# DCASE-REPO/DESED_task

Measured on AMD Instinct MI355X. Metric: 10s-clips/sec CRNN mean-teacher train @batch48, higher is better.
Workload: dtype f32 (fp32 storage and accumulation; the dense contractions of the wide layers run as split-bf16 MFMA, 3 bf16 products per fp32 product, fp32-level accuracy; everything else exact f32)

## Files before the change

### desed_task_amd/csrc/sed_conv.hip

```cpp
#include "sed_common.h"

__global__ __launch_bounds__(256) void pack_weights_kernel(const float* __restrict__ W, float* __restrict__ Wf,
                                                           float* __restrict__ Wd, int COUT, int CIN) {
    const int i = blockIdx.x * 256 + threadIdx.x;
    if (i >= COUT * CIN * 9) return;
    const int b = i % 3, a = (i / 3) % 3, ci = (i / 9) % CIN, co = i / (9 * CIN);
    const float w = W[i];
    Wf[((a * 3 + b) * CIN + ci) * COUT + co] = w;
    if (Wd) Wd[(((2 - a) * 3 + (2 - b)) * COUT + co) * CIN + ci] = w;
}
SED_API int sed_conv_pack_weights(const float* W, float* Wf, float* Wd, int COUT, int CIN, void* stream) {
    const int n = COUT * CIN * 9;
    SED_LAUNCH(pack_weights_kernel, dim3((n + 255) / 256), dim3(256), 0, (hipStream_t)stream, W, Wf, Wd, COUT, CIN);
    return sed_check_launch();
}
struct PackJobs {
    const float* W[8];
    float* Wf[8];
    float* Wd[8];
    int cout[8], cin[8], start[9];
    int n;
};
__global__ __launch_bounds__(256) void pack_weights_multi_kernel(PackJobs jobs) {
    const int i = blockIdx.x * 256 + threadIdx.x;
    if (i >= jobs.start[jobs.n]) return;
    int j = 0;
#pragma unroll
    for (int q = 1; q < 8; ++q) j += (q < jobs.n && i >= jobs.start[q]) ? 1 : 0;
    const int e = i - jobs.start[j], COUT = jobs.cout[j], CIN = jobs.cin[j];
    const int b = e % 3, a = (e / 3) % 3, ci = (e / 9) % CIN, co = e / (9 * CIN);
    const float w = jobs.W[j][e];
    jobs.Wf[j][((a * 3 + b) * CIN + ci) * COUT + co] = w;
    if (jobs.Wd[j]) jobs.Wd[j][(((2 - a) * 3 + (2 - b)) * COUT + co) * CIN + ci] = w;
}
SED_API int sed_conv_pack_multi(int n, const void* const* W, void* const* Wf, void* const* Wd, const int* cout, const int* cin,
                                   void* stream) {
    if (n < 1 || n > 8) return SED_ERR_ARG;
    PackJobs jobs;
    int tot = 0;
    for (int j = 0; j < n; ++j) {
        jobs.W[j] = (const float*)W[j]; jobs.Wf[j] = (float*)Wf[j]; jobs.Wd[j] = Wd ? (float*)Wd[j] : nullptr;
        jobs.cout[j] = cout[j]; jobs.cin[j] = cin[j]; jobs.start[j] = tot;
        tot += cout[j] * cin[j] * 9;
    }
    for (int j = n; j < 8; ++j) { jobs.W[j] = nullptr; jobs.Wf[j] = nullptr; jobs.Wd[j] = nullptr; jobs.cout[j] = 0; jobs.cin[j] = 0; jobs.start[j] = tot; }
    jobs.start[n] = tot;
    jobs.start[8] = tot;
    jobs.n = n;
    SED_LAUNCH(pack_weights_multi_kernel, dim3((tot + 255) / 256), dim3(256), 0, (hipStream_t)stream, jobs);
    return sed_check_launch();
}

__global__ __launch_bounds__(1024) void wgrad_reduce_kernel(const float* __restrict__ parts, float* __restrict__ dW, int nparts,
                                                            int COUT, int CIN) {
    __shared__ float4 red[64][16];
    const int tid = threadIdx.x, col = tid & 15, grp = tid >> 4, G = blockDim.x >> 4;
    const int j = blockIdx.x * 64 + 4 * col;
    const int n = 9 * CIN * COUT;
    float4 acc = make_float4(0.f, 0.f, 0.f, 0.f);
    if (j < n) {
#pragma unroll 4
        for (int p = grp; p < nparts; p += G) {
            const float4 v = *(const float4*)(parts + (size_t)p * n + j);
            acc.x += v.x; acc.y += v.y; acc.z += v.z; acc.w += v.w;
        }
    }
    red[grp][col] = acc;
    __syncthreads();
    if (grp == 0 && j < n) {
        for (int g = 1; g < G; ++g) { const float4 v = red[g][col]; acc.x += v.x; acc.y += v.y; acc.z += v.z; acc.w += v.w; }
        const int co = j % COUT, ci = (j / COUT) % CIN, tap = j / (COUT * CIN);
        float* d = dW + ((size_t)co * CIN + ci) * 9 + tap;
        d[0] = acc.x; d[(size_t)CIN * 9] = acc.y; d[(size_t)2 * CIN * 9] = acc.z; d[(size_t)3 * CIN * 9] = acc.w;
    }
}
static inline int wgrad_parts(int CIN, int COUT, int B, int T, int F) {
    if (CIN <= 32) {
        const int TF = F >= 32 ? 32 : F, TR = 128 / TF;
        const int ntiles = B * ((T + TR - 1) / TR) * (F / TF);
        int cap = CIN <= 16 ? 1024 : 512;
        if (sed_tuning[SED_TUNE_WGRAD_CAP] > 0) cap = sed_tuning[SED_TUNE_WGRAD_CAP];
        return ntiles < cap ? ntiles : cap;
    }
    const int ntiles = (B * T * F + 63) / 64;
    return ntiles < 56 ? ntiles : 56;
}
static inline bool wgrad_row_ok(int CIN, int COUT, int F) {
    return F >= 8 && 64 % F == 0 && COUT == 128 && (CIN == 64 || CIN == 128);
}
static inline int wgrad_row_parts(int CIN, int B, int T, int F) {
    const int ntiles = (B * T * F + 63) / 64, cap = CIN == 64 ? 168 : 84;
    return ntiles < cap ? ntiles : cap;
}
SED_API long long sed_conv_wgrad_scratch_floats(int B, int T, int F, int CIN, int COUT) {
    int parts = wgrad_parts(CIN, COUT, B, T, F);
    if (wgrad_row_ok(CIN, COUT, F) && wgrad_row_parts(CIN, B, T, F) > parts) parts = wgrad_row_parts(CIN, B, T, F);
    return (long long)parts * 9 * CIN * COUT;
}

#define CONV_THREADS(COUT) ((COUT) >= 64 ? 512 : 256)

template <int CIN, int COUT, int TF, int MP = 128>
struct ConvCfg {
    static constexpr int TR = MP / TF;
    static constexpr int PW = TF + 2, PH = TR + 2, PP = PW * PH;
    static constexpr int CK = CIN < 32 ? CIN : 32;
    static constexpr int CKP = CK + 1;
    static constexpr int NCH = CIN / CK;
    static constexpr int NT = (COUT + 31) / 32;
    static constexpr int WM = MP / 32;
    static constexpr int THREADS = CONV_THREADS(COUT);
    static constexpr int WN = THREADS / 64 / WM;
    static constexpr int NTW = NT / WN;
    static_assert(NTW >= 1 && NTW * WN == NT, "wave split must tile COUT");
    static constexpr int WCH = CK * COUT;
    static constexpr int PATCH_F = (PP * CKP + 3) & ~3;
    static constexpr int SMEM = (PATCH_F + 2 * WCH) * 4;
};

template <int CIN, int COUT, int TF, bool STATS, int MP = 128>
__global__ __launch_bounds__(CONV_THREADS(COUT)) void conv3x3_kernel(const float* __restrict__ x, const float* __restrict__ Wp,
                                                      const float* __restrict__ bias, float* __restrict__ y,
                                                      float* __restrict__ partial, int B, int T, int F) {
    using Cfg = ConvCfg<CIN, COUT, TF, MP>;
    constexpr int TR = Cfg::TR, PW = Cfg::PW, PP = Cfg::PP, CK = Cfg::CK, CKP = Cfg::CKP, NCH = Cfg::NCH, NT = Cfg::NT,
                  WCH = Cfg::WCH, NTW = Cfg::NTW, THREADS = Cfg::THREADS, WM = Cfg::WM;
    SED_DYN_SMEM(smem);
    float* patch = (float*)smem;
    float* wbuf = patch + Cfg::PATCH_F;
    const int tid = threadIdx.x, lane = tid & 63, w = (tid >> 6) % WM, wn = (tid >> 6) / WM, lo = lane & 31, hi = lane >> 5;
    const int ftiles = F / TF, ttiles = (T + TR - 1) / TR;
    const int bid = blockIdx.x;
    const int ft = bid % ftiles, tt = (bid / ftiles) % ttiles, b = bid / (ftiles * ttiles);
    const int t0 = tt * TR, f0 = ft * TF;
    const int p = 32 * w + lo;
    const int abase = ((p / TF) * PW + (p % TF)) * CKP + hi;

    f32x16 acc[NTW];
#pragma unroll
    for (int nt = 0; nt < NTW; ++nt) acc[nt] = f32x16_zero();

    constexpr int WV = (WCH / 4 + THREADS - 1) / THREADS;
    float4 wreg[WV];

    for (int cc = 0; cc < NCH; ++cc) {
        constexpr int V = CK / 4;
        {
            constexpr int NLD = (PP * V + THREADS - 1) / THREADS;
            float4 ld[NLD];
#pragma unroll
            for (int u = 0; u < NLD; ++u) {
                const int idx = tid + THREADS * u;
                const int pix = idx / V, v = idx - pix * V;
                const int i = pix / PW, j = pix - i * PW;
                const int t = t0 - 1 + i, f = f0 - 1 + j;
                ld[u] = make_float4(0.f, 0.f, 0.f, 0.f);
                if (idx < PP * V && t >= 0 && t < T && f >= 0 && f < F)
                    ld[u] = *(const float4*)(x + (((size_t)b * T + t) * F + f) * CIN + cc * CK + 4 * v);
            }
#pragma unroll
            for (int u = 0; u < NLD; ++u) {
                const int idx = tid + THREADS * u;
                if (idx < PP * V) {
                    const int pix = idx / V, v = idx - pix * V;
                    float* d = patch + pix * CKP + 4 * v;
                    d[0] = ld[u].x; d[1] = ld[u].y; d[2] = ld[u].z; d[3] = ld[u].w;
                }
            }
        }
        {
            const float4* src = (const float4*)(Wp + ((size_t)0 * CIN + cc * CK) * COUT);
#pragma unroll
            for (int i = 0; i < WV; ++i) {
                const int idx = tid + THREADS * i;
                if (idx < WCH / 4) ((float4*)wbuf)[idx] = src[idx];
            }
        }
        __syncthreads();
#pragma unroll 1
        for (int tap = 0; tap < 9; ++tap) {
            if (tap + 1 < 9) {
                const float4* src = (const float4*)(Wp + ((size_t)(tap + 1) * CIN + cc * CK) * COUT);
#pragma unroll
                for (int i = 0; i < WV; ++i) {
                    const int idx = tid + THREADS * i;
                    float4 wv = make_float4(0.f, 0.f, 0.f, 0.f);
                    if (idx < WCH / 4) wv = src[idx];
                    wreg[i] = wv;
                }
            }
            const float* wb = wbuf + (tap & 1) * WCH;
            const float* ap = patch + abase + ((tap / 3) * PW + (tap % 3)) * CKP;
#pragma unroll
            for (int k = 0; k < CK; k += 2) {
                const float av = ap[k];
#pragma unroll
                for (int nt = 0; nt < NTW; ++nt) {
                    const float bv = (COUT >= 32 || lo < COUT) ? wb[(k + hi) * COUT + (wn * NTW + nt) * 32 + lo] : 0.f;
                    acc[nt] = mfma32(av, bv, acc[nt]);
                }
            }
            if (tap + 1 < 9) {
                float4* dst = (float4*)(wbuf + ((tap + 1) & 1) * WCH);
#pragma unroll
                for (int i = 0; i < WV; ++i) {
                    const int idx = tid + THREADS * i;
                    if (idx < WCH / 4) dst[idx] = wreg[i];
                }
            }
            __syncthreads();
        }
    }
    float* red = wbuf;
#pragma unroll
    for (int nt = 0; nt < NTW; ++nt) {
        const int co = (wn * NTW + nt) * 32 + lo;
        const float bv = (bias != nullptr && co < COUT) ? bias[co] : 0.f;
        float s = 0.f, s2 = 0.f;
#pragma unroll
        for (int r = 0; r < 16; ++r) {
            const int pp = 32 * w + mfma32_row(r, lane);
            const int t = t0 + pp / TF, f = f0 + pp % TF;
            if (t < T && co < COUT) {
                const float v = acc[nt][r] + bv;
                y[(((size_t)b * T + t) * F + f) * COUT + co] = v;
                s += v;
                s2 += v * v;
            }
        }
        if (STATS) {
            s += __shfl_xor(s, 32);
            s2 += __shfl_xor(s2, 32);
            if (hi == 0) {
                red[(w * 2 + 0) * (NT * 32) + co] = s;
                red[(w * 2 + 1) * (NT * 32) + co] = s2;
            }
        }
    }
    if (STATS) {
        __syncthreads();
        if (tid < 2 * COUT) {
            const int which = tid / COUT, co = tid - which * COUT;
            float v = 0.f;
#pragma unroll
            for (int ww = 0; ww < WM; ++ww) v += red[(ww * 2 + which) * (NT * 32) + co];
// ... 328 lines not shown
    bf16_split2(a, b, h.x, l.x);
    bf16_split2(c, d, h.y, l.y);
    *(uint2*)hi_row = h;
    *(uint2*)lo_row = l;
}
__device__ __forceinline__ void wgb_store_block(const float4 v0, const float4 v1, const float4 v2, const float4 v3,
                                                unsigned short* __restrict__ hi_plane, unsigned short* __restrict__ lo_plane,
                                                int cq, int pq, int RS) {
    const int r0 = 4 * cq, f0 = (r0 ^ cq) & 7;
    const int o0 = r0 * RS + 4 * (pq ^ (2 * f0)), o1 = (r0 + 1) * RS + 4 * (pq ^ (2 * (f0 ^ 1)));
    const int o2 = (r0 + 2) * RS + 4 * (pq ^ (2 * (f0 ^ 2))), o3 = (r0 + 3) * RS + 4 * (pq ^ (2 * (f0 ^ 3)));
    wgb_store_row(v0.x, v1.x, v2.x, v3.x, hi_plane + o0, lo_plane + o0);
    wgb_store_row(v0.y, v1.y, v2.y, v3.y, hi_plane + o1, lo_plane + o1);
    wgb_store_row(v0.z, v1.z, v2.z, v3.z, hi_plane + o2, lo_plane + o2);
    wgb_store_row(v0.w, v1.w, v2.w, v3.w, hi_plane + o3, lo_plane + o3);
}

template <int CIN, int COUT>
__global__ __launch_bounds__(256) void conv_wgrad_bf16_kernel(const float* __restrict__ x, const float* __restrict__ dy,
                                                              float* __restrict__ dWp, int B, int T, int F) {
    using Cfg = WgbCfg<CIN, COUT>;
    constexpr int KT = Cfg::KT, RS = Cfg::RS, WN = Cfg::WN, MTW = Cfg::MTW, NTW = Cfg::NTW, NBX = Cfg::NBX, NBD = Cfg::NBD;
    SED_DYN_SMEM(smem);
    unsigned short* xh = (unsigned short*)smem;
    unsigned short* xl = xh + CIN * RS;
    unsigned short* dh = xl + CIN * RS;
    unsigned short* dl = dh + COUT * RS;
    const int tid = threadIdx.x, lane = tid & 63, w = tid >> 6, lo = lane & 31, hi = lane >> 5;
    const int wn = w % WN, wm = w / WN;
    const int tap = blockIdx.y, da = tap / 3 - 1, db = tap % 3 - 1;
    const int npix = B * T * F;
    const int ntiles = (npix + KT - 1) / KT;
    const int fsh = 31 - __builtin_clz(F);

    f32x16 acc[MTW][NTW];
#pragma unroll
    for (int m = 0; m < MTW; ++m)
#pragma unroll
        for (int n = 0; n < NTW; ++n) acc[m][n] = f32x16_zero();

    float4 rx[NBX * 4], rd[NBD * 4];
    unsigned okx = 0, okd = 0;
    static_assert(NBX * 4 <= 32 && NBD * 4 <= 32, "validity masks");
    auto load_tile = [&](int tile) {
        const int p0 = tile * KT;
        okx = 0; okd = 0;
#pragma unroll
        for (int u = 0; u < NBX; ++u) {
            const int blk = tid + 256 * u, cq = (blk >> 1) % (CIN / 4), pq = (blk & 1) + 2 * ((blk >> 1) / (CIN / 4));
#pragma unroll
            for (int j = 0; j < 4; ++j) {
                const int p = p0 + 4 * pq + j, pc = p < npix ? p : 0;
                const int f = pc & (F - 1), tt = pc >> fsh, t = tt % T, bb = tt / T;
                const int t2 = t + da, f2 = f + db;
                const bool ok = p < npix && t2 >= 0 && t2 < T && f2 >= 0 && f2 < F;
                okx |= (ok ? 1u : 0u) << (4 * u + j);
                const int t2c = t2 < 0 ? 0 : (t2 >= T ? T - 1 : t2), f2c = f2 < 0 ? 0 : (f2 >= F ? F - 1 : f2);
                rx[4 * u + j] = *(const float4*)(x + (((size_t)bb * T + t2c) * F + f2c) * CIN + 4 * cq);
            }
        }
#pragma unroll
        for (int u = 0; u < NBD; ++u) {
            const int blk = tid + 256 * u, cq = (blk >> 1) % (COUT / 4), pq = (blk & 1) + 2 * ((blk >> 1) / (COUT / 4));
#pragma unroll
            for (int j = 0; j < 4; ++j) {
                const int p = p0 + 4 * pq + j;
                okd |= (p < npix ? 1u : 0u) << (4 * u + j);
                rd[4 * u + j] = *(const float4*)(dy + (size_t)(p < npix ? p : 0) * COUT + 4 * cq);
            }
        }
    };
    auto store_tile = [&]() {
#pragma unroll
        for (int i = 0; i < NBX * 4; ++i) if (!((okx >> i) & 1u)) rx[i] = make_float4(0.f, 0.f, 0.f, 0.f);
#pragma unroll
        for (int i = 0; i < NBD * 4; ++i) if (!((okd >> i) & 1u)) rd[i] = make_float4(0.f, 0.f, 0.f, 0.f);
#pragma unroll
        for (int u = 0; u < NBX; ++u) {
            const int blk = tid + 256 * u;
            wgb_store_block(rx[4 * u], rx[4 * u + 1], rx[4 * u + 2], rx[4 * u + 3], xh, xl, (blk >> 1) % (CIN / 4),
                            (blk & 1) + 2 * ((blk >> 1) / (CIN / 4)), RS);
        }
#pragma unroll
        for (int u = 0; u < NBD; ++u) {
            const int blk = tid + 256 * u;
            wgb_store_block(rd[4 * u], rd[4 * u + 1], rd[4 * u + 2], rd[4 * u + 3], dh, dl, (blk >> 1) % (COUT / 4),
                            (blk & 1) + 2 * ((blk >> 1) / (COUT / 4)), RS);
        }
    };

    int tile = blockIdx.x;
    if (tile < ntiles) load_tile(tile);
    for (; tile < ntiles; tile += gridDim.x) {
        __syncthreads();
        store_tile();
        __syncthreads();
        if (tile + (int)gridDim.x < ntiles) load_tile(tile + gridDim.x);
#pragma unroll
        for (int ks = 0; ks < KT / 16; ++ks) {
            const int oct = 2 * ks + hi;
            s16x8 a_hi[MTW], a_lo[MTW];
#pragma unroll
            for (int m = 0; m < MTW; ++m) {
                const int row = (wm * MTW + m) * 32 + lo;
                const int off = row * RS + 8 * (oct ^ ((row ^ (row >> 2)) & 7));
                a_hi[m] = *(const s16x8*)(xh + off);
                a_lo[m] = *(const s16x8*)(xl + off);
            }
#pragma unroll
            for (int n = 0; n < NTW; ++n) {
                const int row = (wn * NTW + n) * 32 + lo;
                const int off = row * RS + 8 * (oct ^ ((row ^ (row >> 2)) & 7));
                const s16x8 b_hi = *(const s16x8*)(dh + off);
                const s16x8 b_lo = *(const s16x8*)(dl + off);
#pragma unroll
                for (int m = 0; m < MTW; ++m) {
                    acc[m][n] = mfma32_bf16(a_lo[m], b_hi, acc[m][n]);
                    acc[m][n] = mfma32_bf16(a_hi[m], b_lo, acc[m][n]);
                    acc[m][n] = mfma32_bf16(a_hi[m], b_hi, acc[m][n]);
                }
            }
        }
    }
    float* part = dWp + ((size_t)blockIdx.x * 9 + tap) * CIN * COUT;
#pragma unroll
    for (int m = 0; m < MTW; ++m)
#pragma unroll
        for (int n = 0; n < NTW; ++n) {
            const int co = (wn * NTW + n) * 32 + lo;
#pragma unroll
            for (int r = 0; r < 16; ++r) part[(size_t)((wm * MTW + m) * 32 + mfma32_row(r, lane)) * COUT + co] = acc[m][n][r];
        }
}

template <int CIN, int COUT>
static int launch_wgrad_bf16(const float* x, const float* dy, float* dWp, int B, int T, int F, hipStream_t s) {
    using Cfg = WgbCfg<CIN, COUT>;
    const int splits = wgrad_parts(CIN, COUT, B, T, F);
    SED_MAX_SMEM((conv_wgrad_bf16_kernel<CIN, COUT>), Cfg::SMEM);
    SED_LAUNCH((conv_wgrad_bf16_kernel<CIN, COUT>), dim3(splits, 9), dim3(256), Cfg::SMEM, s, x, dy, dWp, B, T, F);
    return sed_check_launch();
}

template <int CIN, int COUT, int COH>
struct WgrCfg {
    static constexpr int KT = 64, RS = 64;
    static constexpr int MT = CIN / 32, NT = COH / 32;
    static constexpr int WM = MT >= 4 ? 2 : 1, WN = 4 / WM;
    static constexpr int MTW = MT / WM, NTW = NT / WN;
    static constexpr int NBX = (KT / 4) * (CIN / 4) / 256, NBD = (KT / 4) * (COH / 4) / 256;
    static constexpr int SMEM = 2 * (CIN + COH) * RS * 2;
    static_assert(NBX >= 1 && NBD >= 1 && MTW * WM == MT && NTW * WN == NT && MTW * NTW == 2, "tile split");
};
template <int CIN, int COUT, int COH>
__global__ __launch_bounds__(256) void conv_wgrad_bf16_row_kernel(const float* __restrict__ x, const float* __restrict__ dy,
                                                                  float* __restrict__ dWp, int B, int T, int F) {
    using Cfg = WgrCfg<CIN, COUT, COH>;
    constexpr int KT = Cfg::KT, RS = Cfg::RS, WN = Cfg::WN, MTW = Cfg::MTW, NTW = Cfg::NTW, NBX = Cfg::NBX, NBD = Cfg::NBD;
    SED_DYN_SMEM(smem);
    unsigned short* xh = (unsigned short*)smem;
    unsigned short* xl = xh + CIN * RS;
    unsigned short* dh = xl + CIN * RS;
    unsigned short* dl = dh + COH * RS;
    const int lane = threadIdx.x & 63, w = threadIdx.x >> 6;
    int tid = threadIdx.x, lo = lane & 31, hi = lane >> 5;
    const int wn = w % WN, wm = w / WN;
    const int da = (int)blockIdx.y - 1, co0 = blockIdx.z * COH;
    const int npix = B * T * F;
    const int ntiles = (npix + KT - 1) / KT;
    const int fsh = 31 - __builtin_clz(F);

    f32x16 acc[3][MTW][NTW];
#pragma unroll
    for (int t3 = 0; t3 < 3; ++t3)
#pragma unroll
        for (int m = 0; m < MTW; ++m)
#pragma unroll
            for (int n = 0; n < NTW; ++n) acc[t3][m][n] = f32x16_zero();

    float4 rx[NBX * 4], rd[NBD * 4];
    unsigned okm = 0;
    auto load_tile = [&](int tile) {
        const int p0 = tile * KT;
        okm = 0;
#pragma unroll
        for (int u = 0; u < NBX; ++u) {
            const int blk = tid + 256 * u, cq = (blk >> 1) % (CIN / 4), pq = (blk & 1) + 2 * ((blk >> 1) / (CIN / 4));
            const int pb = p0 + 4 * pq, pbc = pb < npix ? pb : 0, tt = pbc >> fsh, t = tt % T, bb = tt / T, t2 = t + da, f = pbc & (F - 1);
            const bool ok = pb < npix && t2 >= 0 && t2 < T;
            okm |= (ok ? 1u : 0u) << u;
            const float* src = x + (((size_t)bb * T + (t2 < 0 ? 0 : (t2 >= T ? T - 1 : t2))) * F + f) * CIN + 4 * cq;
#pragma unroll
            for (int j = 0; j < 4; ++j) rx[4 * u + j] = *(const float4*)(src + (size_t)j * CIN);
        }
#pragma unroll
        for (int u = 0; u < NBD; ++u) {
            const int blk = tid + 256 * u, cq = (blk >> 1) % (COH / 4), pq = (blk & 1) + 2 * ((blk >> 1) / (COH / 4));
            const int pb = p0 + 4 * pq;
            okm |= (pb < npix ? 1u : 0u) << (16 + u);
            const float* src = dy + (size_t)(pb < npix ? pb : 0) * COUT + co0 + 4 * cq;
#pragma unroll
            for (int j = 0; j < 4; ++j) rd[4 * u + j] = *(const float4*)(src + (size_t)j * COUT);
        }
    };
    auto store_tile = [&]() {
#pragma unroll
        for (int u = 0; u < NBX; ++u)
            if (!((okm >> u) & 1u)) {
#pragma unroll
                for (int j = 0; j < 4; ++j) rx[4 * u + j] = make_float4(0.f, 0.f, 0.f, 0.f);
            }
#pragma unroll
        for (int u = 0; u < NBD; ++u)
            if (!((okm >> (16 + u)) & 1u)) {
#pragma unroll
                for (int j = 0; j < 4; ++j) rd[4 * u + j] = make_float4(0.f, 0.f, 0.f, 0.f);
            }
#pragma unroll
        for (int u = 0; u < NBX; ++u) {
            const int blk = tid + 256 * u;
            wgb_store_block(rx[4 * u], rx[4 * u + 1], rx[4 * u + 2], rx[4 * u + 3], xh, xl, (blk >> 1) % (CIN / 4),
                            (blk & 1) + 2 * ((blk >> 1) / (CIN / 4)), RS);
        }
#pragma unroll
        for (int u = 0; u < NBD; ++u) {
            const int blk = tid + 256 * u;
            wgb_store_block(rd[4 * u], rd[4 * u + 1], rd[4 * u + 2], rd[4 * u + 3], dh, dl, (blk >> 1) % (COH / 4),
                            (blk & 1) + 2 * ((blk >> 1) / (COH / 4)), RS);
        }
    };
    auto shift_m1 = [](const uint4 c, unsigned prev3) {
        uint4 r;
        r.x = sed_alignbit(c.x, prev3, 16); r.y = sed_alignbit(c.y, c.x, 16); r.z = sed_alignbit(c.z, c.y, 16); r.w = sed_alignbit(c.w, c.z, 16);
        return r;
    };
    auto shift_p1 = [](const uint4 c, unsigned next0) {
        uint4 r;
        r.x = sed_alignbit(c.y, c.x, 16); r.y = sed_alignbit(c.z, c.y, 16); r.z = sed_alignbit(c.w, c.z, 16); r.w = sed_alignbit(next0, c.w, 16);
        return r;
    };

    int tile = blockIdx.x;
    if (tile < ntiles) load_tile(tile);
    for (; tile < ntiles; tile += gridDim.x) {
        sed_opaque(tid); sed_opaque(lo); sed_opaque(hi);
        __syncthreads();
        store_tile();
        __syncthreads();
        if (tile + (int)gridDim.x < ntiles) load_tile(tile + gridDim.x);
#pragma unroll
        for (int ks = 0; ks < KT / 16; ++ks) {
            const int oct = 2 * ks + hi;
            const bool first = ((8 * oct) & (F - 1)) == 0, last = ((8 * oct + 8) & (F - 1)) == 0;
            s16x8 a_hi[3][MTW], a_lo[3][MTW];
#pragma unroll
            for (int m = 0; m < MTW; ++m) {
                const int row = (wm * MTW + m) * 32 + lo, sw = (row ^ (row >> 2)) & 7;
                const int off = row * RS + 8 * (oct ^ sw);
                const int offp = row * RS + 8 * (((oct + 7) & 7) ^ sw) + 6, offn = row * RS + 8 * (((oct + 1) & 7) ^ sw);
                const uint4 ch = *(const uint4*)(xh + off), cl = *(const uint4*)(xl + off);
                const unsigned ph = first ? 0u : *(const unsigned*)(xh + offp), pl = first ? 0u : *(const unsigned*)(xl + offp);
                const unsigned nh = last ? 0u : *(const unsigned*)(xh + offn), nl = last ? 0u : *(const unsigned*)(xl + offn);
                a_hi[0][m] = __builtin_bit_cast(s16x8, shift_m1(ch, ph)); a_lo[0][m] = __builtin_bit_cast(s16x8, shift_m1(cl, pl));
                a_hi[1][m] = __builtin_bit_cast(s16x8, ch);               a_lo[1][m] = __builtin_bit_cast(s16x8, cl);
                a_hi[2][m] = __builtin_bit_cast(s16x8, shift_p1(ch, nh)); a_lo[2][m] = __builtin_bit_cast(s16x8, shift_p1(cl, nl));
            }
#pragma unroll
            for (int n = 0; n < NTW; ++n) {
                const int row = (wn * NTW + n) * 32 + lo;
                const int off = row * RS + 8 * (oct ^ ((row ^ (row >> 2)) & 7));
                const s16x8 b_hi = *(const s16x8*)(dh + off);
                const s16x8 b_lo = *(const s16x8*)(dl + off);
#pragma unroll
                for (int t3 = 0; t3 < 3; ++t3)
#pragma unroll
                    for (int m = 0; m < MTW; ++m) {
                        acc[t3][m][n] = mfma32_bf16(a_lo[t3][m], b_hi, acc[t3][m][n]);
                        acc[t3][m][n] = mfma32_bf16(a_hi[t3][m], b_lo, acc[t3][m][n]);
                        acc[t3][m][n] = mfma32_bf16(a_hi[t3][m], b_hi, acc[t3][m][n]);
                    }
            }
        }
    }
#pragma unroll
    for (int t3 = 0; t3 < 3; ++t3) {
        float* part = dWp + ((size_t)blockIdx.x * 9 + 3 * (da + 1) + t3) * CIN * COUT;
#pragma unroll
        for (int m = 0; m < MTW; ++m)
#pragma unroll
            for (int n = 0; n < NTW; ++n) {
                const int co = co0 + (wn * NTW + n) * 32 + lo;
#pragma unroll
                for (int r = 0; r < 16; ++r) part[(size_t)((wm * MTW + m) * 32 + mfma32_row(r, lane)) * COUT + co] = acc[t3][m][n][r];
            }
    }
}
template <int CIN, int COUT, int COH>
static int launch_wgrad_bf16_row(const float* x, const float* dy, float* dWp, int B, int T, int F, int splits, hipStream_t s) {
    using Cfg = WgrCfg<CIN, COUT, COH>;
    SED_MAX_SMEM((conv_wgrad_bf16_row_kernel<CIN, COUT, COH>), Cfg::SMEM);
    SED_LAUNCH((conv_wgrad_bf16_row_kernel<CIN, COUT, COH>), dim3(splits, 3, COUT / COH), dim3(256), Cfg::SMEM, s, x, dy, dWp, B, T, F);
    return sed_check_launch();
}

template <int CIN, int COUT, int TF>
struct WgaCfg {
    static constexpr int TR = 128 / TF, PW = TF + 2, PH = TR + 2, PP = PW * PH;
    static constexpr int NT = COUT / 32, WN = NT >= 2 ? 2 : 1, WK = 4 / WN, NTW = NT / WN;
    static constexpr int SMEM = (PP * CIN + 128 * COUT) * 4;
};
template <int CIN, int COUT, int TF>
__global__ __launch_bounds__(256) void conv_wgrad_alltaps_kernel(const float* __restrict__ x, const float* __restrict__ dy,
                                                                 float* __restrict__ dWp, int B, int T, int F) {
    using Cfg = WgaCfg<CIN, COUT, TF>;
    constexpr int TR = Cfg::TR, PW = Cfg::PW, PP = Cfg::PP, WN = Cfg::WN, WK = Cfg::WK, NTW = Cfg::NTW;
    static_assert(CIN <= 32, "narrow layers only");
    SED_DYN_SMEM(smem);
    float* xs = (float*)smem;
    float* ds = xs + PP * CIN;
    const int tid = threadIdx.x, lane = tid & 63, w = tid >> 6, lo = lane & 31, hi = lane >> 5;
    const int wn = w % WN, wk = w / WN;
    const int ftiles = F / TF, ttiles = (T + TR - 1) / TR, ntiles = B * ttiles * ftiles;
    constexpr bool M16 = CIN == 16;
    constexpr int NT16 = COUT / 16, WK16 = 4;
    f32x16 acc[M16 ? 1 : 9][M16 ? 1 : NTW];
    f32x4 acc16[M16 ? 9 : 1][M16 ? NT16 : 1];
#pragma unroll
    for (int tp = 0; tp < (M16 ? 1 : 9); ++tp)
#pragma unroll
        for (int n = 0; n < (M16 ? 1 : NTW); ++n) acc[tp][n] = f32x16_zero();
#pragma unroll
    for (int tp = 0; tp < (M16 ? 9 : 1); ++tp)
#pragma unroll
        for (int n = 0; n < (M16 ? NT16 : 1); ++n) acc16[tp][n] = f32x4{0.f, 0.f, 0.f, 0.f};

    constexpr int NX = (PP * (CIN / 4) + 255) / 256, ND = 128 * (COUT / 4) / 256;
    float4 lx[NX], ldy[ND];
    auto load_tile = [&](int tile_) {
        const int ft = tile_ % ftiles, tt = (tile_ / ftiles) % ttiles, b = tile_ / (ftiles * ttiles);
        const int t0 = tt * TR, f0 = ft * TF;
#pragma unroll
        for (int u = 0; u < NX; ++u) {
            const int idx = tid + 256 * u, pix = idx / (CIN / 4), v = idx - pix * (CIN / 4);
            const int i = pix / PW, j = pix - i * PW;
            const int t = t0 - 1 + i, f = f0 - 1 + j;
            float4 val = make_float4(0.f, 0.f, 0.f, 0.f);
            if (idx < PP * (CIN / 4) && t >= 0 && t < T && f >= 0 && f < F)
                val = *(const float4*)(x + (((size_t)b * T + t) * F + f) * CIN + 4 * v);
            lx[u] = val;
        }
#pragma unroll
        for (int u = 0; u < ND; ++u) {
            const int idx = tid + 256 * u, p = idx / (COUT / 4), v = idx - p * (COUT / 4);
            const int t = t0 + p / TF, f = f0 + p % TF;
            float4 val = make_float4(0.f, 0.f, 0.f, 0.f);
            if (t < T) val = *(const float4*)(dy + (((size_t)b * T + t) * F + f) * COUT + 4 * v);
            ldy[u] = val;
        }
    };
    int tile = blockIdx.x;
    if (tile < ntiles) load_tile(tile);
    for (; tile < ntiles; tile += gridDim.x) {
        __syncthreads();
#pragma unroll
        for (int u = 0; u < NX; ++u) {
            const int idx = tid + 256 * u;
            if (idx < PP * (CIN / 4)) *(float4*)(xs + (idx / (CIN / 4)) * CIN + 4 * (idx % (CIN / 4))) = lx[u];
        }
#pragma unroll
        for (int u = 0; u < ND; ++u) {
            const int idx = tid + 256 * u;
            *(float4*)(ds + (idx / (COUT / 4)) * COUT + 4 * (idx % (COUT / 4))) = ldy[u];
        }
        __syncthreads();
        if (tile + (int)gridDim.x < ntiles) load_tile(tile + gridDim.x);
        if (M16) {
            constexpr int KS16 = 128 / WK16;
            const int i16 = lane & 15, g16 = lane >> 4;
#pragma unroll 2
            for (int k = w * KS16; k < (w + 1) * KS16; k += 4) {
                const int p = k + g16;
                const int pb = (p / TF) * PW + (p % TF);
                float bv16[NT16];
#pragma unroll
                for (int n = 0; n < NT16; ++n) bv16[n] = ds[p * COUT + n * 16 + i16];
#pragma unroll
                for (int tp = 0; tp < 9; ++tp) {
                    const float av = xs[(pb + (tp / 3) * PW + (tp % 3)) * CIN + i16];
#pragma unroll
                    for (int n = 0; n < NT16; ++n) acc16[M16 ? tp : 0][M16 ? n : 0] = mfma16(av, bv16[n], acc16[M16 ? tp : 0][M16 ? n : 0]);
                }
            }
            continue;
        }
        constexpr int KS = 128 / WK;
#pragma unroll 2
        for (int k = wk * KS; k < (wk + 1) * KS; k += 2) {
            const int p = k + hi;
            const int pb = (p / TF) * PW + (p % TF);
            float bv[NTW];
#pragma unroll
            for (int n = 0; n < NTW; ++n) bv[n] = ds[p * COUT + (wn * NTW + n) * 32 + lo];
#pragma unroll
            for (int tp = 0; tp < 9; ++tp) {
                const float av = (CIN >= 32 || lo < CIN) ? xs[(pb + (tp / 3) * PW + (tp % 3)) * CIN + lo] : 0.f;
#pragma unroll
                for (int n = 0; n < NTW; ++n) acc[tp][n] = mfma32(av, bv[n], acc[tp][n]);
            }
        }
    }
    float* red = (float*)smem;
    float* part = dWp + (size_t)blockIdx.x * 9 * CIN * COUT;
    constexpr int TG = 5;
    if (M16) {
        const int i16 = lane & 15, g16 = lane >> 4;
#pragma unroll
        for (int g0 = 0; g0 < 9; g0 += TG) {
            for (int round = 0; round < WK16; ++round) {
                __syncthreads();
                if (w == round) {
#pragma unroll
                    for (int tp = g0; tp < g0 + TG && tp < 9; ++tp)
#pragma unroll
                        for (int n = 0; n < NT16; ++n)
#pragma unroll
                            for (int r = 0; r < 4; ++r) {
                                float* d = red + ((tp - g0) * CIN + 4 * g16 + r) * COUT + n * 16 + i16;
                                const float v = acc16[M16 ? tp : 0][M16 ? n : 0][r];
                                *d = (round == 0) ? v : *d + v;
                            }
                }
            }
            __syncthreads();
            const int ntp = (9 - g0) < TG ? (9 - g0) : TG;
            for (int idx = tid; idx < ntp * CIN * COUT; idx += 256) part[(size_t)g0 * CIN * COUT + idx] = red[idx];
        }
        return;
    }
#pragma unroll
    for (int g0 = 0; g0 < 9; g0 += TG) {
        for (int round = 0; round < WK; ++round) {
            __syncthreads();
            if (wk == round) {
#pragma unroll
                for (int tp = g0; tp < g0 + TG && tp < 9; ++tp)
#pragma unroll
                    for (int n = 0; n < NTW; ++n) {
                        const int co = (wn * NTW + n) * 32 + lo;
#pragma unroll
                        for (int r = 0; r < 16; ++r) {
                            const int ci = mfma32_row(r, lane);
                            if (ci < CIN) {
                                float* d = red + ((tp - g0) * CIN + ci) * COUT + co;
                                *d = (round == 0) ? acc[tp][n][r] : *d + acc[tp][n][r];
// ... 106 lines not shown
                    unsigned short* dst = xp + (4 * v + c) * XS + i * TF + 4 * cq;
#pragma unroll
                    for (int sft = 0; sft < 3; ++sft) {
                        uint2 hv, lv;
                        hv.x = ph[sft]; hv.y = ph[sft + 2];
                        lv.x = pl[sft]; lv.y = pl[sft + 2];
                        *(uint2*)(dst + (2 * sft) * XPLANE) = hv;
                        *(uint2*)(dst + (2 * sft + 1) * XPLANE) = lv;
                    }
                }
            }
        }
#pragma unroll
        for (int u = 0; u < NDU; ++u) {
            const int it = tid + 256 * u, cq = it % 8, v = (it / 8) % VD, r = it / (8 * VD);
#pragma unroll
            for (int c = 0; c < 4; ++c) {
                uint2 hv, lv;
                bf16_split2(comp(ld[u][0], c), comp(ld[u][1], c), hv.x, lv.x);
                bf16_split2(comp(ld[u][2], c), comp(ld[u][3], c), hv.y, lv.y);
                unsigned short* dst = dp + (4 * v + c) * DS + r * TF + 4 * cq;
                *(uint2*)dst = hv;
                *(uint2*)(dst + DPLANE) = lv;
            }
        }
    };
    int tile = blockIdx.x;
    if (tile < ntiles) load_tile(tile);
    for (; tile < ntiles; tile += gridDim.x) {
        sed_opaque(tid); sed_opaque(lo); sed_opaque(hi); sed_opaque(i16); sed_opaque(g);
        __syncthreads();
        if (!(WGN_ABL & 4)) store_tile();
        else if (lx[0][0].x + ld[0][0].x == 123.456f) xp[tid] = 1;
        __syncthreads();
        if (tile + (int)gridDim.x < ntiles) load_tile(tile + gridDim.x);
        if (WGN_ABL & 2) continue;
        if (M16) {
            s16x8 bh[2], bl[2], ah[9], al[9];
#pragma unroll
            for (int nt = 0; nt < 2; ++nt) {
                const unsigned short* bp = dp + (16 * nt + i16) * DS + w * TF + 8 * g;
                bh[nt] = *(const s16x8*)bp;
                bl[nt] = *(const s16x8*)(bp + DPLANE);
            }
#pragma unroll
            for (int tp = 0; tp < 9; ++tp) {
                const unsigned short* ap = xp + (2 * (tp % 3)) * XPLANE + i16 * XS + (w + tp / 3) * TF + 8 * g;
                ah[tp] = *(const s16x8*)ap;
                al[tp] = *(const s16x8*)(ap + XPLANE);
            }
            sed_sched_fence();
#pragma unroll
            for (int tp = 0; tp < 9; ++tp)
#pragma unroll
                for (int nt = 0; nt < 2; ++nt) {
                    f32x4 a = acc16[M16 ? tp : 0][nt];
                    if (WGN_ABL & 1) { a[0] += (float)(al[tp][0] + bh[nt][1] + ah[tp][2] + bl[nt][3]); }
                    else {
                    a = mfma16_bf16(al[tp], bh[nt], a);
                    a = mfma16_bf16(ah[tp], bl[nt], a);
                    a = mfma16_bf16(ah[tp], bh[nt], a);
                    }
                    acc16[M16 ? tp : 0][nt] = a;
                }
        } else {
            const int wn = w & 1, wk = w >> 1;
            s16x8 bh[2], bl[2], ah[2][9], al[2][9];
            auto fetch = [&](int k4, int buf) {
                const int ks = 4 * wk + k4, r = ks >> 1, c0 = 16 * (ks & 1) + 8 * hi;
                const unsigned short* bp = dp + (32 * wn + lo) * DS + r * TF + c0;
                bh[buf] = *(const s16x8*)bp;
                bl[buf] = *(const s16x8*)(bp + DPLANE);
#pragma unroll
                for (int tp = 0; tp < 9; ++tp) {
                    const unsigned short* ap = xp + (2 * (tp % 3)) * XPLANE + lo * XS + (r + tp / 3) * TF + c0;
                    ah[buf][tp] = *(const s16x8*)ap;
                    al[buf][tp] = *(const s16x8*)(ap + XPLANE);
                }
            };
            fetch(0, 0);
            sed_sched_fence();
#pragma unroll
            for (int k4 = 0; k4 < 4; ++k4) {
                const int cur = k4 & 1;
                if (k4 + 1 < 4) fetch(k4 + 1, cur ^ 1);
#pragma unroll
                for (int tp = 0; tp < 9; ++tp) {
                    f32x16 a = acc[M16 ? 0 : tp];
                    if (WGN_ABL & 1) { a[0] += (float)(al[cur][tp][0] + bh[cur][1] + ah[cur][tp][2] + bl[cur][3]); }
                    else {
                    a = mfma32_bf16(al[cur][tp], bh[cur], a);
                    a = mfma32_bf16(ah[cur][tp], bl[cur], a);
                    a = mfma32_bf16(ah[cur][tp], bh[cur], a);
                    }
                    acc[M16 ? 0 : tp] = a;
                }
                sed_sched_fence();
            }
        }
    }
    float* red = (float*)smem;
    float* part = dWp + (size_t)blockIdx.x * 9 * CIN * COUT;
    if (M16) {
        for (int round = 0; round < 4; ++round) {
            __syncthreads();
            if (w == round) {
#pragma unroll
                for (int tp = 0; tp < 9; ++tp)
#pragma unroll
                    for (int nt = 0; nt < 2; ++nt)
#pragma unroll
                        for (int r = 0; r < 4; ++r) {
                            float* d = red + (tp * CIN + 4 * g + r) * COUT + 16 * nt + i16;
                            const float v = acc16[M16 ? tp : 0][nt][r];
                            *d = round == 0 ? v : *d + v;
                        }
            }
        }
    } else {
        const int wn = w & 1, wk = w >> 1;
        for (int round = 0; round < 2; ++round) {
            __syncthreads();
            if (wk == round) {
#pragma unroll
                for (int tp = 0; tp < 9; ++tp)
#pragma unroll
                    for (int r = 0; r < 16; ++r) {
                        float* d = red + (tp * CIN + mfma32_row(r, lane)) * COUT + 32 * wn + lo;
                        const float v = acc[M16 ? 0 : tp][r];
                        *d = round == 0 ? v : *d + v;
                    }
            }
        }
    }
    __syncthreads();
    for (int idx = threadIdx.x; idx < 9 * CIN * COUT; idx += 256) part[idx] = red[idx];
}
template <int CIN, int COUT>
static int launch_wgrad_alltaps_bf16(const float* x, const float* dy, float* dWp, int B, int T, int F, int grid, hipStream_t s) {
    using Cfg = WgnCfg<CIN, COUT>;
    SED_MAX_SMEM((conv_wgrad_alltaps_bf16_kernel<CIN, COUT>), Cfg::SMEM);
    SED_LAUNCH((conv_wgrad_alltaps_bf16_kernel<CIN, COUT>), dim3(grid), dim3(256), Cfg::SMEM, s, x, dy, dWp, B, T, F);
    return sed_check_launch();
}

static int conv_wgrad_impl(const float* x, const float* dy, float* dWp, float* dW, int B, int T, int F, int CIN, int COUT,
                           bool split_bf16, void* stream) {
    hipStream_t s = (hipStream_t)stream;
    int rc = SED_ERR_UNSUPPORTED;
    const int TF = conv_tf(F);
    if (F % TF != 0 || (F & (F - 1)) != 0) return SED_ERR_UNSUPPORTED;
    int nparts = wgrad_parts(CIN, COUT, B, T, F);
    if (split_bf16 && TF == 32 && sed_tuning[SED_TUNE_WGRAD_NARROW] != 1 && ((CIN == 16 && COUT == 32) || (CIN == 32 && COUT == 64))) {
        const int capb = sed_tuning[SED_TUNE_WGRAD_CAP] > 0 ? sed_tuning[SED_TUNE_WGRAD_CAP] : (CIN == 16 ? 512 : 256);
        if (nparts > capb) nparts = capb;
        if (CIN == 16) rc = launch_wgrad_alltaps_bf16<16, 32>(x, dy, dWp, B, T, F, nparts, s);
        else rc = launch_wgrad_alltaps_bf16<32, 64>(x, dy, dWp, B, T, F, nparts, s);
    }
#define WGA_CASE(ci, co, tf) if (rc != SED_OK && CIN == ci && COUT == co && TF == tf) rc = launch_wgrad_alltaps<ci, co, tf>(x, dy, dWp, B, T, F, s);
    WGA_CASE(16, 32, 32) WGA_CASE(16, 32, 16) WGA_CASE(16, 32, 8) WGA_CASE(32, 64, 32) WGA_CASE(32, 64, 16) WGA_CASE(32, 64, 8)
    WGA_CASE(32, 64, 4)
#undef WGA_CASE
    if (rc != SED_OK && split_bf16 && wgrad_row_ok(CIN, COUT, F) && sed_tuning[SED_TUNE_WGRAD_WIDE] != 1) {
        nparts = wgrad_row_parts(CIN, B, T, F);
        if (CIN == 64) rc = launch_wgrad_bf16_row<64, 128, 128>(x, dy, dWp, B, T, F, nparts, s);
        else rc = launch_wgrad_bf16_row<128, 128, 64>(x, dy, dWp, B, T, F, nparts, s);
    }
#define WG_CASE(ci, co)                                                                                        \
    if (rc != SED_OK && CIN == ci && COUT == co)                                                               \
        rc = split_bf16 ? launch_wgrad_bf16<ci, co>(x, dy, dWp, B, T, F, s) : launch_wgrad<ci, co>(x, dy, dWp, B, T, F, s);
    WG_CASE(64, 128) WG_CASE(128, 128)
#undef WG_CASE
    if (rc != SED_OK) return rc;
    const int n = COUT * CIN * 9;
    SED_LAUNCH(wgrad_reduce_kernel, dim3((n + 63) / 64), dim3(nparts >= 256 ? 1024 : 256), 0, s, (const float*)dWp, dW, nparts, COUT, CIN);
    return sed_check_launch();
}
SED_API int sed_conv_wgrad(const float* x, const float* dy, float* dWp, float* dW, int B, int T, int F, int CIN, int COUT,
                              void* stream) {
    return conv_wgrad_impl(x, dy, dWp, dW, B, T, F, CIN, COUT, false, stream);
}
SED_API int sed_conv_wgrad_bf16x3(const float* x, const float* dy, float* dWp, float* dW, int B, int T, int F, int CIN,
                                     int COUT, void* stream) {
    return conv_wgrad_impl(x, dy, dWp, dW, B, T, F, CIN, COUT, true, stream);
}

__global__ __launch_bounds__(256) void conv0_wgrad_kernel(const float* __restrict__ x, const int* __restrict__ bounds,
                                                          const float* __restrict__ dyz, const float* __restrict__ y,
                                                          const float* __restrict__ stats, const float* __restrict__ gamma,
                                                          const float* __restrict__ dgamma, const float* __restrict__ dbeta,
                                                          float* __restrict__ dW, int B, int T, int F, int tiles_t, int fuse_bn,
                                                          int training, float inv_count) {
    constexpr int C = 16;
    __shared__ float tile[(C0_TR + 2) * (128 + 2)];
    __shared__ float red[4][144];
    const int tid = threadIdx.x, PW = F + 2, cq = tid & 3;
    float acc[4][9];
#pragma unroll
    for (int c = 0; c < 4; ++c)
#pragma unroll
        for (int k = 0; k < 9; ++k) acc[c][k] = 0.f;
    float mean[4], istd[4], m1[4], m2[4];
#pragma unroll
    for (int c = 0; c < 4; ++c) {
        const int ch = 4 * cq + c;
        mean[c] = fuse_bn ? stats[ch] : 0.f;
        istd[c] = fuse_bn ? stats[C + ch] : 1.f;
        m1[c] = (fuse_bn && training) ? gamma[ch] * dbeta[ch] * inv_count : 0.f;
        m2[c] = (fuse_bn && training) ? gamma[ch] * dgamma[ch] * inv_count : 0.f;
    }
    const int ntiles = B * tiles_t;
    for (int tl = blockIdx.x; tl < ntiles; tl += gridDim.x) {
        const int b = tl / tiles_t, t0 = (tl - b * tiles_t) * C0_TR;
        int mf0 = 0, mf1 = 0, mt0 = 0, mt1 = 0;
        if (bounds) { mf0 = bounds[4 * b]; mf1 = bounds[4 * b + 1]; mt0 = bounds[4 * b + 2]; mt1 = bounds[4 * b + 3]; }
        __syncthreads();
        for (int idx = tid; idx < (C0_TR + 2) * PW; idx += 256) {
            const int i = idx / PW, j = idx - i * PW;
            const int t = t0 - 1 + i, f = j - 1;
            float v = 0.f;
            if (t >= 0 && t < T && f >= 0 && f < F) {
                v = x[((size_t)b * T + t) * F + f];
                if ((f >= mf0 && f < mf1) || (t >= mt0 && t < mt1)) v = 0.f;
            }
            tile[idx] = v;
        }
        __syncthreads();
        for (int p = tid >> 2; p < C0_TR * F; p += 64) {
            const int pr = p / F, pc = p - pr * F, t = t0 + pr;
            if (t < T) {
                const size_t off = (((size_t)b * T + t) * F + pc) * C + 4 * cq;
                const float4 gz = *(const float4*)(dyz + off);
                float g[4] = {gz.x, gz.y, gz.z, gz.w};
                if (fuse_bn) {
                    const float4 yv = *(const float4*)(y + off);
                    const float yy[4] = {yv.x, yv.y, yv.z, yv.w};
#pragma unroll
                    for (int c = 0; c < 4; ++c) g[c] = istd[c] * (g[c] - m1[c] - (yy[c] - mean[c]) * istd[c] * m2[c]);
                }
#pragma unroll
                for (int a = 0; a < 3; ++a)
#pragma unroll
                    for (int bb = 0; bb < 3; ++bb) {
                        const float xv = tile[(pr + a) * PW + pc + bb];
#pragma unroll
                        for (int c = 0; c < 4; ++c) acc[c][a * 3 + bb] = fmaf(xv, g[c], acc[c][a * 3 + bb]);
                    }
            }
        }
    }
#pragma unroll
    for (int c = 0; c < 4; ++c)
#pragma unroll
        for (int k = 0; k < 9; ++k) {
            float v = acc[c][k];
#pragma unroll
            for (int m = 4; m <= 32; m <<= 1) v += __shfl_xor(v, m);
            if ((tid & 63) < 4) red[tid >> 6][(4 * cq + c) * 9 + k] = v;
        }
    __syncthreads();
    if (tid < 144) atomicAdd(dW + tid, red[0][tid] + red[1][tid] + red[2][tid] + red[3][tid]);
}
SED_API int sed_conv0_wgrad(const float* x, const int* bounds, const float* dyz, const float* y, const float* stats,
                               const float* gamma, const float* dgamma, const float* dbeta, float* dW, float* dbias, int B, int T,
                               int F, int COUT, int fuse_bn, int training, void* stream) {
    if (COUT != 16 || F > 128 || F < 1) return SED_ERR_UNSUPPORTED;
    hipStream_t s = (hipStream_t)stream;
    sed_zero4(s, dW, 16 * 9, fuse_bn ? dbias : nullptr, fuse_bn ? 16 : 0, nullptr, 0, nullptr, 0);
    if (B <= 0 || T <= 0) return SED_OK;
    if (fuse_bn && !training) return SED_ERR_UNSUPPORTED;
    const int tiles_t = (T + C0_TR - 1) / C0_TR;
    int grid = B * tiles_t;
    if (grid > 1024) grid = 1024;
    SED_LAUNCH(conv0_wgrad_kernel, dim3(grid), dim3(256), 0, s, x, bounds, dyz, y, stats, gamma, dgamma, dbeta, dW, B, T, F, tiles_t,
               fuse_bn, training, 1.0f / ((float)B * (float)T * (float)F));
    return sed_check_launch();
}
```

Measured before the change: 16370.

## Extend row-wise bf16 wgrad kernel to small F and balance split counts

Adds a SMALLF variant of the row-based split-bf16 weight-gradient kernel that handles F=2/4 by loading pixel pairs and masking the tap shifts at row boundaries. Wide layers with small frequency width can then use the MFMA row kernel instead of the generic fallback. Split counts are now chosen so the tiles divide evenly across splits, which removes tail imbalance. The grid is flattened with split-major interleaving of tap/channel slots for better scheduling. This adds more kernel variants and boundary-mask logic that could introduce correctness risk.

```diff
diff --git a/desed_task_amd/csrc/sed_conv.hip b/desed_task_amd/csrc/sed_conv.hip
--- a/desed_task_amd/csrc/sed_conv.hip
+++ b/desed_task_amd/csrc/sed_conv.hip
@@ -74,23 +74,39 @@
         d[0] = acc.x; d[(size_t)CIN * 9] = acc.y; d[(size_t)2 * CIN * 9] = acc.z; d[(size_t)3 * CIN * 9] = acc.w;
     }
 }
+static inline int wgrad_splits(int ntiles, int max_splits) {
+    if (ntiles <= max_splits) return ntiles < 1 ? 1 : ntiles;
+    const int per0 = (ntiles + max_splits - 1) / max_splits;
+    for (int per = per0; per < 2 * per0; ++per)
+        if (ntiles % per == 0) return ntiles / per;
+    return (ntiles + per0 - 1) / per0;
+}
+static inline int wgrad_narrow_tiles(int B, int T, int F) {
+    const int TF = F >= 32 ? 32 : F, TR = 128 / TF;
+    return B * ((T + TR - 1) / TR) * (F / TF);
+}
 static inline int wgrad_parts(int CIN, int COUT, int B, int T, int F) {
     if (CIN <= 32) {
-        const int TF = F >= 32 ? 32 : F, TR = 128 / TF;
-        const int ntiles = B * ((T + TR - 1) / TR) * (F / TF);
+        const int ntiles = wgrad_narrow_tiles(B, T, F);
         int cap = CIN <= 16 ? 1024 : 512;
         if (sed_tuning[SED_TUNE_WGRAD_CAP] > 0) cap = sed_tuning[SED_TUNE_WGRAD_CAP];
-        return ntiles < cap ? ntiles : cap;
-    }
-    const int ntiles = (B * T * F + 63) / 64;
-    return ntiles < 56 ? ntiles : 56;
+        return CIN <= 16 ? (ntiles < cap ? ntiles : cap) : wgrad_splits(ntiles, cap);
+    }
+    return wgrad_splits((B * T * F + 63) / 64, sed_tuning[SED_TUNE_WGRAD_CAP] > 0 ? sed_tuning[SED_TUNE_WGRAD_CAP] : 56);
+}
+static inline int wgrad_narrow_bf16_parts(int CIN, int B, int T, int F) {
+    const int ntiles = wgrad_narrow_tiles(B, T, F);
+    const int cap = sed_tuning[SED_TUNE_WGRAD_CAP] > 0 ? sed_tuning[SED_TUNE_WGRAD_CAP] : (CIN == 16 ? 512 : 256);
+    if (CIN == 16) return ntiles < cap ? ntiles : cap;
+    return wgrad_splits(ntiles, cap);
 }
 static inline bool wgrad_row_ok(int CIN, int COUT, int F) {
-    return F >= 8 && 64 % F == 0 && COUT == 128 && (CIN == 64 || CIN == 128);
+    return F >= 2 && 64 % F == 0 && COUT == 128 && (CIN == 64 || CIN == 128);
 }
 static inline int wgrad_row_parts(int CIN, int B, int T, int F) {
-    const int ntiles = (B * T * F + 63) / 64, cap = CIN == 64 ? 168 : 84;
-    return ntiles < cap ? ntiles : cap;
+    int cap = CIN == 64 ? 168 : (F <= 4 ? 39 : 84);
+    if (sed_tuning[SED_TUNE_WGRAD_CAP] > 0) cap = sed_tuning[SED_TUNE_WGRAD_CAP];
+    return wgrad_splits((B * T * F + 63) / 64, cap);
 }
 SED_API long long sed_conv_wgrad_scratch_floats(int B, int T, int F, int CIN, int COUT) {
     int parts = wgrad_parts(CIN, COUT, B, T, F);
@@ -725,9 +741,9 @@
     static constexpr int SMEM = 2 * (CIN + COH) * RS * 2;
     static_assert(NBX >= 1 && NBD >= 1 && MTW * WM == MT && NTW * WN == NT && MTW * NTW == 2, "tile split");
 };
-template <int CIN, int COUT, int COH>
-__global__ __launch_bounds__(256) void conv_wgrad_bf16_row_kernel(const float* __restrict__ x, const float* __restrict__ dy,
-                                                                  float* __restrict__ dWp, int B, int T, int F) {
+template <int CIN, int COUT, int COH, bool SMALLF>
+__device__ __forceinline__ void conv_wgrad_bf16_row_body(const float* __restrict__ x, const float* __restrict__ dy,
+                                                         float* __restrict__ dWp, int B, int T, int F, int nsplit) {
     using Cfg = WgrCfg<CIN, COUT, COH>;
     constexpr int KT = Cfg::KT, RS = Cfg::RS, WN = Cfg::WN, MTW = Cfg::MTW, NTW = Cfg::NTW, NBX = Cfg::NBX, NBD = Cfg::NBD;
     SED_DYN_SMEM(smem);
@@ -738,7 +754,10 @@
     const int lane = threadIdx.x & 63, w = threadIdx.x >> 6;
     int tid = threadIdx.x, lo = lane & 31, hi = lane >> 5;
     const int wn = w % WN, wm = w / WN;
-    const int da = (int)blockIdx.y - 1, co0 = blockIdx.z * COH;
+    constexpr int Q = 3 * (COUT / COH);
+    const int slot = (int)blockIdx.x >> 3, split = 8 * (slot / Q) + ((int)blockIdx.x & 7), jq = slot % Q;
+    if (split >= nsplit) return;
+    const int da = jq % 3 - 1, co0 = (jq / 3) * COH;
     const int npix = B * T * F;
     const int ntiles = (npix + KT - 1) / KT;
     const int fsh = 31 - __builtin_clz(F);
@@ -753,12 +772,25 @@
 
     float4 rx[NBX * 4], rd[NBD * 4];
     unsigned okm = 0;
+    static_assert(2 * NBX <= 16 && 2 * NBD <= 16, "validity masks");
     auto load_tile = [&](int tile) {
         const int p0 = tile * KT;
         okm = 0;
 #pragma unroll
         for (int u = 0; u < NBX; ++u) {
             const int blk = tid + 256 * u, cq = (blk >> 1) % (CIN / 4), pq = (blk & 1) + 2 * ((blk >> 1) / (CIN / 4));
+            if constexpr (SMALLF) {
+#pragma unroll
+                for (int h = 0; h < 2; ++h) {
+                    const int pp = p0 + 4 * pq + 2 * h, ppc = pp < npix ? pp : 0, tt = ppc >> fsh, t = tt % T, bb = tt / T, t2 = t + da;
+                    const bool ok = pp < npix && t2 >= 0 && t2 < T;
+                    okm |= (ok ? 1u : 0u) << (2 * u + h);
+                    const float* src = x + (((size_t)bb * T + (t2 < 0 ? 0 : (t2 >= T ? T - 1 : t2))) * F + (ppc & (F - 1))) * CIN + 4 * cq;
+                    rx[4 * u + 2 * h] = *(const float4*)src;
+                    rx[4 * u + 2 * h + 1] = *(const float4*)(src + CIN);
+                }
+                continue;
+            }
             const int pb = p0 + 4 * pq, pbc = pb < npix ? pb : 0, tt = pbc >> fsh, t = tt % T, bb = tt / T, t2 = t + da, f = pbc & (F - 1);
             const bool ok = pb < npix && t2 >= 0 && t2 < T;
             okm |= (ok ? 1u : 0u) << u;
@@ -770,6 +802,17 @@
         for (int u = 0; u < NBD; ++u) {
             const int blk = tid + 256 * u, cq = (blk >> 1) % (COH / 4), pq = (blk & 1) + 2 * ((blk >> 1) / (COH / 4));
             const int pb = p0 + 4 * pq;
+            if constexpr (SMALLF) {
+#pragma unroll
+                for (int h = 0; h < 2; ++h) {
+                    const int pp = pb + 2 * h;
+                    okm |= (pp < npix ? 1u : 0u) << (16 + 2 * u + h);
+                    const float* src = dy + (size_t)(pp < npix ? pp : 0) * COUT + co0 + 4 * cq;
+                    rd[4 * u + 2 * h] = *(const float4*)src;
+                    rd[4 * u + 2 * h + 1] = *(const float4*)(src + COUT);
+                }
+                continue;
+            }
             okm |= (pb < npix ? 1u : 0u) << (16 + u);
             const float* src = dy + (size_t)(pb < npix ? pb : 0) * COUT + co0 + 4 * cq;
 #pragma unroll
@@ -777,18 +820,27 @@
         }
     };
     auto store_tile = [&]() {
-#pragma unroll
-        for (int u = 0; u < NBX; ++u)
-            if (!((okm >> u) & 1u)) {
-#pragma unroll
-                for (int j = 0; j < 4; ++j) rx[4 * u + j] = make_float4(0.f, 0.f, 0.f, 0.f);
-            }
-#pragma unroll
-        for (int u = 0; u < NBD; ++u)
-            if (!((okm >> (16 + u)) & 1u)) {
-#pragma unroll
-                for (int j = 0; j < 4; ++j) rd[4 * u + j] = make_float4(0.f, 0.f, 0.f, 0.f);
-            }
+        if constexpr (SMALLF) {
+#pragma unroll
+            for (int i = 0; i < 2 * NBX; ++i)
+                if (!((okm >> i) & 1u)) rx[2 * i] = rx[2 * i + 1] = make_float4(0.f, 0.f, 0.f, 0.f);
+#pragma unroll
+            for (int i = 0; i < 2 * NBD; ++i)
+                if (!((okm >> (16 + i)) & 1u)) rd[2 * i] = rd[2 * i + 1] = make_float4(0.f, 0.f, 0.f, 0.f);
+        } else {
+#pragma unroll
+            for (int u = 0; u < NBX; ++u)
+                if (!((okm >> u) & 1u)) {
+#pragma unroll
+                    for (int j = 0; j < 4; ++j) rx[4 * u + j] = make_float4(0.f, 0.f, 0.f, 0.f);
+                }
+#pragma unroll
+            for (int u = 0; u < NBD; ++u)
+                if (!((okm >> (16 + u)) & 1u)) {
+#pragma unroll
+                    for (int j = 0; j < 4; ++j) rd[4 * u + j] = make_float4(0.f, 0.f, 0.f, 0.f);
+                }
+        }
 #pragma unroll
         for (int u = 0; u < NBX; ++u) {
             const int blk = tid + 256 * u;
@@ -813,14 +865,26 @@
         return r;
     };
 
-    int tile = blockIdx.x;
+    const unsigned keep_hi = F == 2 ? 0xffff0000u : 0xffffffffu, keep_lo = F == 2 ? 0x0000ffffu : 0xffffffffu;
+    auto shift_m1_rows = [&](const uint4 c) {
+        uint4 r = shift_m1(c, 0u);
+        r.y &= keep_hi; r.z &= 0xffff0000u; r.w &= keep_hi;
+        return r;
+    };
+    auto shift_p1_rows = [&](const uint4 c) {
+        uint4 r = shift_p1(c, 0u);
+        r.x &= keep_lo; r.y &= 0x0000ffffu; r.z &= keep_lo;
+        return r;
+    };
+
+    int tile = split;
     if (tile < ntiles) load_tile(tile);
-    for (; tile < ntiles; tile += gridDim.x) {
+    for (; tile < ntiles; tile += nsplit) {
         sed_opaque(tid); sed_opaque(lo); sed_opaque(hi);
         __syncthreads();
         store_tile();
         __syncthreads();
-        if (tile + (int)gridDim.x < ntiles) load_tile(tile + gridDim.x);
+        if (tile + nsplit < ntiles) load_tile(tile + nsplit);
 #pragma unroll
         for (int ks = 0; ks < KT / 16; ++ks) {
             const int oct = 2 * ks + hi;
@@ -830,6 +894,13 @@
             for (int m = 0; m < MTW; ++m) {
                 const int row = (wm * MTW + m) * 32 + lo, sw = (row ^ (row >> 2)) & 7;
                 const int off = row * RS + 8 * (oct ^ sw);
+                if constexpr (SMALLF) {
+                    const uint4 ch = *(const uint4*)(xh + off), cl = *(const uint4*)(xl + off);
+                    a_hi[0][m] = __builtin_bit_cast(s16x8, shift_m1_rows(ch)); a_lo[0][m] = __builtin_bit_cast(s16x8, shift_m1_rows(cl));
+                    a_hi[1][m] = __builtin_bit_cast(s16x8, ch);                a_lo[1][m] = __builtin_bit_cast(s16x8, cl);
+                    a_hi[2][m] = __builtin_bit_cast(s16x8, shift_p1_rows(ch)); a_lo[2][m] = __builtin_bit_cast(s16x8, shift_p1_rows(cl));
+                    continue;
+                }
                 const int offp = row * RS + 8 * (((oct + 7) & 7) ^ sw) + 6, offn = row * RS + 8 * (((oct + 1) & 7) ^ sw);
                 const uint4 ch = *(const uint4*)(xh + off), cl = *(const uint4*)(xl + off);
                 const unsigned ph = first ? 0u : *(const unsigned*)(xh + offp), pl = first ? 0u : *(const unsigned*)(xl + offp);
@@ -857,7 +928,7 @@
     }
 #pragma unroll
     for (int t3 = 0; t3 < 3; ++t3) {
-        float* part = dWp + ((size_t)blockIdx.x * 9 + 3 * (da + 1) + t3) * CIN * COUT;
+        float* part = dWp + ((size_t)split * 9 + 3 * (da + 1) + t3) * CIN * COUT;
 #pragma unroll
         for (int m = 0; m < MTW; ++m)
 #pragma unroll
@@ -867,12 +938,28 @@
                 for (int r = 0; r < 16; ++r) part[(size_t)((wm * MTW + m) * 32 + mfma32_row(r, lane)) * COUT + co] = acc[t3][m][n][r];
             }
     }
+}
+template <int CIN, int COUT, int COH>
+__global__ __launch_bounds__(256) void conv_wgrad_bf16_row_kernel(const float* __restrict__ x, const float* __restrict__ dy,
+                                                                  float* __restrict__ dWp, int B, int T, int F, int nsplit) {
+    conv_wgrad_bf16_row_body<CIN, COUT, COH, false>(x, dy, dWp, B, T, F, nsplit);
+}
+template <int CIN, int COUT, int COH>
+__global__ __launch_bounds__(256) void conv_wgrad_bf16_rowf_kernel(const float* __restrict__ x, const float* __restrict__ dy,
+                                                                   float* __restrict__ dWp, int B, int T, int F, int nsplit) {
+    conv_wgrad_bf16_row_body<CIN, COUT, COH, true>(x, dy, dWp, B, T, F, nsplit);
 }
 template <int CIN, int COUT, int COH>
 static int launch_wgrad_bf16_row(const float* x, const float* dy, float* dWp, int B, int T, int F, int splits, hipStream_t s) {
     using Cfg = WgrCfg<CIN, COUT, COH>;
-    SED_MAX_SMEM((conv_wgrad_bf16_row_kernel<CIN, COUT, COH>), Cfg::SMEM);
-    SED_LAUNCH((conv_wgrad_bf16_row_kernel<CIN, COUT, COH>), dim3(splits, 3, COUT / COH), dim3(256), Cfg::SMEM, s, x, dy, dWp, B, T, F);
+    const dim3 grid(8 * 3 * (COUT / COH) * ((splits + 7) / 8));
+    if (F <= 4) {
+        SED_MAX_SMEM((conv_wgrad_bf16_rowf_kernel<CIN, COUT, COH>), Cfg::SMEM);
+        SED_LAUNCH((conv_wgrad_bf16_rowf_kernel<CIN, COUT, COH>), grid, dim3(256), Cfg::SMEM, s, x, dy, dWp, B, T, F, splits);
+    } else {
+        SED_MAX_SMEM((conv_wgrad_bf16_row_kernel<CIN, COUT, COH>), Cfg::SMEM);
+        SED_LAUNCH((conv_wgrad_bf16_row_kernel<CIN, COUT, COH>), grid, dim3(256), Cfg::SMEM, s, x, dy, dWp, B, T, F, splits);
+    }
     return sed_check_launch();
 }
 
@@ -1285,8 +1372,7 @@
     if (F % TF != 0 || (F & (F - 1)) != 0) return SED_ERR_UNSUPPORTED;
     int nparts = wgrad_parts(CIN, COUT, B, T, F);
     if (split_bf16 && TF == 32 && sed_tuning[SED_TUNE_WGRAD_NARROW] != 1 && ((CIN == 16 && COUT == 32) || (CIN == 32 && COUT == 64))) {
-        const int capb = sed_tuning[SED_TUNE_WGRAD_CAP] > 0 ? sed_tuning[SED_TUNE_WGRAD_CAP] : (CIN == 16 ? 512 : 256);
-        if (nparts > capb) nparts = capb;
+        nparts = wgrad_narrow_bf16_parts(CIN, B, T, F);
         if (CIN == 16) rc = launch_wgrad_alltaps_bf16<16, 32>(x, dy, dWp, B, T, F, nparts, s);
         else rc = launch_wgrad_alltaps_bf16<32, 64>(x, dy, dWp, B, T, F, nparts, s);
     }
```

Measured after the change: 16530 (median of 6 runs). No clear change (+1.0%).
